# NickDrake117/GNNkeras

Hardware: AMD Instinct MI355X
Metric: node-state updates/s (arcs x iterations / s), forward Loop (higher is better)
Workload: dtype f32; 1 GPU; C4 Erdos-Renyi 1000000 nodes / 10000000 arcs, state_dim=64, max_iteration=50, threshold=0 (k=50), node-focused, average aggregation, BN+Dense(159->64,selu) state net

## Files before the change

gnnkeras_amd/_native.py:

```python
from __future__ import annotations

import ctypes as C
import os
import subprocess

import torch

HERE = os.path.dirname(os.path.abspath(__file__))
CSRC = os.path.join(HERE, 'csrc')
LIB_PATH = os.environ.get('GNNKERAS_AMD_LIB') or os.path.join(CSRC, 'libgnnloop.so')

GNN_ABI_VERSION = 10
GNN_MAX_LAYERS = 8
GNN_MAX_TYPES = 8

ACTIVATIONS = {'linear': 0, None: 0, 'relu': 1, 'selu': 2, 'tanh': 3, 'sigmoid': 4, 'elu': 5, 'softplus': 6,
               'softmax': 7}
FOCUS = {'n': 0, 'a': 1, 'g': 2}
FLAG_UNFUSED = 1
FLAG_NO_EARLY_EXIT = 2
FLAG_FUSED_GEN_MASK = 7 << 4
FLAG_TRAIN_HIDDEN_SMALL = 1 << 8
XC_FILL, XC_VALID = 0, 1
FLAG_FUSED_GEN2, FLAG_FUSED_GEN4, FLAG_FUSED_GEN5, FLAG_FUSED_GEN6, FLAG_FUSED_GEN7 = 2 << 4, 4 << 4, 5 << 4, 6 << 4, 7 << 4

EXPORTS = ['gnn_last_error', 'gnn_last_status', 'gnn_last_kernel_name', 'gnn_abi_version', 'gnn_struct_size', 'gnn_loop_workspace_bytes', 'gnn_loop_forward', 'gnn_loop_groups_supported', 'gnn_loop_group_max_nodes', 'gnn_aggregate',
           'gnn_loop_xc_applies', 'gnn_loop_route_name', 'gnn_train_xc_applies',
           'gnn_mlp_workspace_bytes', 'gnn_mlp_forward', 'gnn_converged', 'gnn_state_step', 'gnn_state_step_agg', 'gnn_state_ld', 'gnn_debug_occupy', 'gnn_debug_occupy_until', 'gnn_debug_expiry_beacon', 'gnn_debug_host_flag',
           'gnn_debug_f4_tile_plan', 'gnn_debug_f4_tile_queue_const', 'gnn_debug_f4_last_tickets',
           'gnn_device_malloc', 'gnn_device_free', 'gnn_ipc_export', 'gnn_ipc_open', 'gnn_ipc_close', 'gnn_shard_iteration_peers', 'gnn_peer_wait', 'gnn_peer_publish', 'gnn_shard_iteration_split_rows',
           'gnn_shard_setup', 'gnn_shard_iteration', 'gnn_shard_output', 'gnn_gather_rows',
           'gnn_shard_can_split', 'gnn_shard_partial', 'gnn_shard_iteration_split',
           'gnn_dense', 'gnn_fold_bn', 'gnn_dense_grad_workspace_bytes', 'gnn_dense_grad', 'gnn_act_grad',
           'gnn_colstats_workspace_bytes', 'gnn_colstats', 'gnn_first_layer_param_grads', 'gnn_bn_input_grad',
           'gnn_scatter_add_rows', 'gnn_axpby', 'gnn_loss_grad', 'gnn_dropout', 'gnn_adam_step', 'gnn_adam_multi', 'gnn_sgd_step',
           'gnn_converged_gated', 'gnn_aggregate_gated', 'gnn_train_workspace_bytes', 'gnn_train_step', 'gnn_train_groups_supported', 'gnn_ragged_copy',
           'gnn_train_step_ex', 'gnn_train_phases_supported', 'gnn_gate_all',
           'gnn_comm_unique_id', 'gnn_comm_create', 'gnn_comm_destroy', 'gnn_shard_loop']
GNN_MAX_SEGMENTS = 6
LOSSES = {'categorical_crossentropy': 0, 'cce': 0, 'binary_crossentropy': 1, 'bce': 1, 'mse': 2,
          'mean_squared_error': 2, 'mae': 3, 'mean_absolute_error': 3}

_f32p = C.POINTER(C.c_float)
_i32p = C.POINTER(C.c_int32)
# ... 200 lines not shown
        l.gnn_shard_iteration_peers.restype = C.c_int
        l.gnn_shard_iteration_peers.argtypes = [C.POINTER(LoopArgs), C.c_void_p, C.c_void_p, C.c_int32, C.c_void_p, C.c_int32, C.c_int32, C.c_void_p, C.c_int32,
                                                C.POINTER(PeerSet)]
        l.gnn_peer_wait.restype = C.c_int
        l.gnn_peer_wait.argtypes = [C.c_void_p, C.c_int32, C.c_int32, C.c_int32, C.c_void_p, C.c_void_p]
        l.gnn_peer_publish.restype = C.c_int
        l.gnn_peer_publish.argtypes = [C.POINTER(PeerSet), C.c_void_p, C.c_void_p, C.c_int64, C.c_int32, C.c_int32, C.c_int32, C.c_void_p]
        l.gnn_debug_host_flag.restype = C.c_int
        l.gnn_debug_host_flag.argtypes = [C.POINTER(C.POINTER(C.c_int32)), C.POINTER(C.c_void_p)]
        l.gnn_debug_f4_tile_plan.restype = None
        l.gnn_debug_f4_tile_plan.argtypes = [C.c_int32, C.c_int32, C.c_int32, C.POINTER(C.c_int32)]
        l.gnn_debug_f4_tile_queue_const.restype = C.c_int32
        l.gnn_debug_f4_tile_queue_const.argtypes = [C.c_int32, C.c_int32]
        l.gnn_debug_f4_last_tickets.restype = C.c_longlong
        l.gnn_debug_f4_last_tickets.argtypes = []
        l.gnn_debug_expiry_beacon.restype = C.c_int
        l.gnn_debug_expiry_beacon.argtypes = [C.POINTER(C.c_void_p), C.c_int32, C.c_void_p]
        l.gnn_state_step_agg.restype = C.c_int
        l.gnn_state_step_agg.argtypes = [C.POINTER(LoopArgs), C.c_void_p, C.c_void_p, C.c_int32, C.c_void_p, C.c_int32, C.c_void_p, C.c_void_p]
        l.gnn_state_ld.restype = C.c_int32
        l.gnn_state_ld.argtypes = [C.c_int32]
        l.gnn_shard_setup.restype = C.c_int
        l.gnn_shard_setup.argtypes = [C.POINTER(LoopArgs)]
        l.gnn_shard_iteration.restype = C.c_int
        l.gnn_shard_iteration.argtypes = [C.POINTER(LoopArgs), C.c_void_p, C.c_void_p, C.c_int32, C.c_void_p, C.c_int32,
                                          C.c_int32, C.c_void_p, C.c_int32]
        l.gnn_shard_output.restype = C.c_int
        l.gnn_shard_output.argtypes = [C.POINTER(LoopArgs), C.c_void_p, C.c_void_p, C.c_int32]
        vp, i32, f32, sz = C.c_void_p, C.c_int32, C.c_float, C.c_size_t
        protos = {
# ... 84 lines not shown
```

gnnkeras_amd/csrc/gnnloop.hip:

```cpp
#include <hip/hip_runtime.h>
#include <stdarg.h>
#include <stddef.h>
#include <stdio.h>
#include <stdlib.h>
#include <string.h>
#include <algorithm>
#include <mutex>
#include <string>
#include <vector>

#include "../../include/gnnloop.h"
#include "kernels_general.hpp"
#include "kernel_state_fused2.hpp"
#include "kernel_state_fused4.hpp"
#include "kernel_state_small.hpp"
#include "kernel_state_mid.hpp"
#include "kernel_state_lds.hpp"
#include "kernel_state_lds_types.hpp"
#include "kernel_state_wide.hpp"
#include "kernels_batch.hpp"
#include "kernels_setup.hpp"
#include "kernel_rowdense.hpp"
#include "kernel_state_xwide.hpp"

// ... 38 lines not shown
    if (S <= 128) {
        int p = 16;
        while (p < S) p <<= 1;
        return p;
    }
    return round_up(S, 4);
}

struct Knobs {
    int pin;
    int flag_pin, env_pin;
    int mid_max_nodes;
    bool prefix_fusion, xwide, rowdense;
    bool xc; int xc_min_nodes;
    bool tile_queue;
};
const Knobs &process_knobs() {
    static const Knobs once = [] {
        Knobs k = {};
        const char *e;
        k.env_pin = (e = getenv("GNN_FUSED_KERNEL")) ? atoi(e) : 0;
        k.mid_max_nodes = (e = getenv("GNN_MID_MAX_NODES")) ? atoi(e) : 36000;
        k.prefix_fusion = !((e = getenv("GNN_PREFIX_FUSION")) && e[0] == '0');
        k.xwide = !((e = getenv("GNN_XWIDE")) && atoi(e) == 0);
        k.rowdense = !((e = getenv("GNN_ROWDENSE")) && e[0] == '0');
        return k;
    }();
    return once;
}
Knobs knobs(int flags) {
    Knobs k = process_knobs();
    k.flag_pin = (flags & GNN_FLAG_FUSED_GEN_MASK) >> 4;
    k.pin = k.flag_pin ? k.flag_pin : k.env_pin;
    const char *e = getenv("GNN_XC"), *m = getenv("GNN_XC_MIN_NODES");
    k.xc = !(e && atoi(e) == 0);
    k.xc_min_nodes = m ? atoi(m) : 196608;
    const char *q = getenv("GNN_F4_TILE_QUEUE");
    k.tile_queue = !(q && atoi(q) == 0);
    return k;
}

struct Carver {
    char *base;
    size_t off = 0;
    explicit Carver(void *b) : base((char *)b) {}
    template <typename T>
    T *take(size_t count) {
        off = (off + 255) & ~(size_t)255;
        T *p = base ? (T *)(base + off) : nullptr;
        off += count * sizeof(T);
        return p;
    }
};
// ... 336 lines not shown
    float *Wx;
    bool xc_ok;
    float *buf[2], *agg;
    float *hid[2]; int ld_hid;
    float *Wf_out, *bf_out;
    float *ohid[2]; int ld_ohid;
    float *out_nodes;
    int *idx_src, *idx_dst;
    size_t bytes;
};

constexpr int GNN_SMALL_MAX_TILES = 512;
constexpr int GNN_LOOP_WORDS = 16 + 32 + gnn::MID_BAR_WORDS;
constexpr int GNN_TQ_WORDS = 8;
inline size_t tq_words(const gnn_loop_args_t &a) { return (size_t)GNN_TQ_WORDS * (size_t)a.max_iteration; }

int state_width(const gnn_loop_args_t &a) { return a.state_dim > 0 ? a.state_dim : a.dim_node_label; }

int make_plan(const gnn_loop_args_t &a, void *ws, Plan &p, bool validate_ptrs) {
    memset(&p, 0, sizeof(p));
    if (a.abi_version != GNN_ABI_VERSION) return fail("abi_version %d != %d", a.abi_version, GNN_ABI_VERSION);
    if (a.n_nodes < 0 || a.n_arcs < 0) return fail("negative graph size");
    if (a.state_dim < 0 || a.max_iteration < 0 || !(a.state_threshold >= 0.0f)) return fail("state_dim, max_iteration, state_threshold must be >= 0");
    p.composite = a.composite != 0;
    p.T = p.composite ? a.n_types : 1;
    if (p.T < 1 || p.T > GNN_MAX_TYPES) return fail("n_types %d out of [1,%d]", p.T, GNN_MAX_TYPES);
    if (p.composite && a.max_iteration < 1) return not_covered("composite GNN requires max_iteration > 0");
    p.N = a.n_nodes; p.E = a.n_arcs; p.L = a.dim_node_label; p.A = a.dim_arc_label;
    p.S = state_width(a);
    if (p.S < 1) return fail("state width is 0 (state_dim == 0 and dim_node_label == 0)");
// ... 75 lines not shown
            TRY(check_csr(a.nodegraph, "nodegraph", a.nodegraph.n_dst, p.M));
        }
        if (a.n_heavy_segments > 0) {
            if (!a.heavy_seg_beg || !a.heavy_seg_end) return fail("heavy_seg_beg / heavy_seg_end is NULL");
            TRY(check_csr(a.adjacency_light, "adjacency_light", p.N, (a.nodes_src ? a.adjacency.n_src : p.N) + a.n_heavy_segments));
        }
        if (p.composite) {
            if (!a.type_nodes && p.N > 0) return fail("type_nodes is NULL");
            if (a.type_offsets[0] != 0 || a.type_offsets[p.T] != p.N) return fail("type_offsets must span [0, n_nodes]");
            for (int t = 0; t < p.T; ++t)
                TRY(check_csr(a.composite_adjacency[t], "composite_adjacency", p.N, a.nodes_src ? a.adjacency.n_src : p.N));
        }
    }

    Carver c(ws);
    p.flags = c.take<int>(a.max_iteration + GNN_LOOP_WORDS + tq_words(a));
    p.err = p.flags ? p.flags + a.max_iteration + 12 : nullptr;
    p.tq = p.flags ? p.flags + a.max_iteration + GNN_LOOP_WORDS : nullptr;
    p.mid_bar = p.flags ? p.flags + ((a.max_iteration + 16 + 31) & ~31) : nullptr;
    p.pred0 = c.take<int>(std::max(GNN_SMALL_MAX_TILES, p.group_tiles));
    p.d_group_tabs = c.take<int>(a.n_groups > 0 ? 4 * ((size_t)a.n_groups + 1) : 0);
    p.set_bar = c.take<unsigned long long>(a.n_groups > 0 ? 2 * (size_t)a.n_groups : 0);
    for (int t = 0; t < p.T; ++t) {
        p.tp[t].Wf = c.take<float>((size_t)a.net_state[t].in_dim * a.net_state[t].units[0]);
        p.tp[t].bf = c.take<float>(a.net_state[t].units[0]);
    }
    p.Wf_out = c.take<float>((size_t)a.net_output.in_dim * a.net_output.units[0]);
    p.bf_out = c.take<float>(a.net_output.units[0]);
    p.agg_arcs = c.take<float>((size_t)p.N * std::max(p.A, 1));
    p.ld_agg_nodes = p.composite ? sum_dt : (a.state_dim > 0 ? p.L : 0);
    p.agg_nodes = c.take<float>((size_t)p.N * std::max(p.ld_agg_nodes, 1));
// ... 114 lines not shown
    LAUNCH_OK();
    return 0;
}
int check_xc_args(const gnn_loop_args_t &a) {
    if (!a.xc) return 0;
    if (((uintptr_t)a.xc & 255) != 0) return fail("xc must be 256-byte aligned");
    if (a.xc_mode != GNN_XC_FILL && a.xc_mode != GNN_XC_VALID) return fail("unknown xc_mode %d", a.xc_mode);
    return 0;
}

int setup_constants(const gnn_loop_args_t &a, const Plan &p, hipStream_t st, bool zero_loop_words = false, bool skip_c = false,
                    const GivenAgg *given = nullptr, bool xc_line = false, bool xc_valid = false) {
    FoldList fl;
    for (int t = 0; t < p.T; ++t) fl.add(a.net_state[t], p.tp[t].Wf, p.tp[t].bf);
    if (a.net_output.kernel[0]) fl.add(a.net_output, p.Wf_out, p.bf_out);
    if (zero_loop_words) { fl.fa.zero_a = p.flags; fl.fa.n_a = a.max_iteration + GNN_LOOP_WORDS + (int)tq_words(a); fl.fa.zero_b = a.k_out; fl.fa.n_b = 1; }
    TRY(launch_fold_list(fl, st));
    if (xc_line) {
        const TypePlan &tp = p.tp[0];
        if (!xc_valid) TRY(fill_constants_line(a, p.N, a.state_dim > 0 ? p.L : 0, p.A, p.Xc, st));
        gnn::PackSegs ps;
        memset(&ps, 0, sizeof(ps));
        ps.n = tp.ncseg;
        for (int s2 = 0; s2 < tp.ncseg && s2 < 3; ++s2) { ps.width[s2] = tp.cseg[s2].width; ps.wrow[s2] = tp.cseg[s2].wrow; }
        const int H = tp.net->units[0];
        gnn::k_pack_wc<<<cdiv(32 * H, 256), 256, 0, st>>>(tp.Wf, tp.bf, H, ps, tp.Wc);
        LAUNCH_OK();
        return 0;
    }
    if (given) {
        if (p.A > 0) TRY(launch_copy2d(nullptr, given->arcs, given->ld_arcs, p.agg_arcs, p.A, p.N, p.A, p.A, st));
// ... 59 lines not shown
    sa.nodes_src = a.nodes_src ? a.nodes_src : a.nodes; sa.ld_nodes_src = a.nodes_src ? a.ld_nodes_src : a.ld_nodes;
    sa.adj = gnn::SetupCsr{a.adjacency.rowptr, a.adjacency.src, a.adjacency.w, a.adjacency.row_scale};
    sa.arc_labels = a.arc_labels; sa.ld_arcs = a.ld_arcs; sa.A = p.A;
    sa.arcnode = gnn::SetupCsr{a.arcnode.rowptr, a.arcnode.src, a.arcnode.w, a.arcnode.row_scale};
    if (a.state_dim > 0) { sa.row_nodes = p.S; sa.row_aggn = 2 * p.S + p.L; sa.row_agga = 2 * p.S + 2 * p.L; }
    else                 { sa.row_agga = 2 * p.S; }
    sa.C = p.C; sa.ldC = p.ldC;
    sa.state0 = a.state_dim > 0 ? a.state0 : a.nodes; sa.ld_s0 = a.state_dim > 0 ? p.S : a.ld_nodes;
    sa.S = p.S; sa.thr = a.state_threshold; sa.pred0 = p.pred0;
    sa.zero_a = p.flags; sa.n_a = a.max_iteration + GNN_LOOP_WORDS; sa.zero_b = a.k_out; sa.n_b = std::max(1, p.n_groups);
    gnn::k_setup_small<<<sa.n_tiles + 1, 256, gnn::setup_small_lds(sa.net.H, 2 * L + p.A, std::max(a.net_state[0].in_dim, a.net_output.in_dim)), st>>>(sa);
    LAUNCH_OK();
    return 0;
}

__device__ long long g_f4_last_tickets;
__global__ void k_fold_error(const int *err, float *k_out, const int *tq, int n_tq) {
    long long s = 0;
    for (int i = threadIdx.x; i < n_tq; i += 64) s += tq[i];
    for (int off = 32; off >= 1; off >>= 1) s += __shfl_xor(s, off, 64);
    if (threadIdx.x == 0) {
        g_f4_last_tickets = s;
        if (*err != 0) *k_out = -1.0e9f;
    }
}

int launch_fold_error(const Plan &p, float *k_out, hipStream_t st, const int *tq = nullptr, int n_tq = 0) {
    if (!k_out || !p.err) return 0;
    k_fold_error<<<1, 64, 0, st>>>(p.err, k_out, tq, n_tq);
    LAUNCH_OK();
    return 0;
}

__global__ void k_arc_endpoints(const int *__restrict__ out_index, const int *__restrict__ arc_src,
                                const int *__restrict__ arc_dst, int M, int *__restrict__ idx_src, int *__restrict__ idx_dst) {
    const int m = blockIdx.x * blockDim.x + threadIdx.x;
    if (m < M) { const int e = out_index[m]; idx_src[m] = arc_src[e]; idx_dst[m] = arc_dst[e]; }
}

int output_stage(const gnn_loop_args_t &a, const Plan &p, hipStream_t st) {
    if (p.M == 0) return 0;
    const bool with_labels = !p.composite && a.state_dim > 0;
    MlpRun r;
    r.mlp = &a.net_output; r.Wf = p.Wf_out; r.bf = p.bf_out;
// ... 71 lines not shown
    r.nseg = 1;
    r.segs[0] = gnn::Seg{p.agg, nullptr, p.SP, (int)m.units[1], 0};
    r.M = p.N;
    r.hid[0] = p.hid[0]; r.hid[1] = p.hid[1]; r.ld_hid = p.ld_hid;
    r.Y = dst; r.ldy = p.SP;
    r.gate = gate;
    if (flag_next) { r.pred_old = src; r.ld_pred = p.SP; r.pred_thr = a.state_threshold; r.pred_flag = flag_next; r.pred_k = k_out; r.pred_kval = k_val; }
    TRY(run_mlp(r, st));
    if (flag_next && !r.pred_fused) TRY(launch_converge(gate, dst, src, p.N, p.S, p.SP, p.SP, a.state_threshold, flag_next, k_out, k_val, st));
    return 0;
}

int iteration_fused(const gnn_loop_args_t &a, const Plan &p, IterKernel kernel, const int *gate, int n_gate, int gate_stride,
                    const float *src, float *dst, int row_base, int *flag_next, float *k_out, float k_val,
                    hipStream_t st, const gnn_csr_t *adj_override = nullptr, const float *agg_init = nullptr,
                    const int *rows_override = nullptr, int count_override = 0, const gnn_peer_set_t *peers = nullptr, int *tile_ctr = nullptr) {
    TRY(launch_heavy(a, p, n_gate == 1 ? gate : nullptr, src, st));
    const gnn_csr_t &adj = adj_override ? *adj_override : iter_adjacency(a, p);
    gnn::Fused2Args fa;
    memset(&fa, 0, sizeof(fa));
    fill_fused_args(fa, a, p, adj);
    fa.gate = n_gate ? gate : nullptr; fa.n_gate = n_gate; fa.gate_stride = gate_stride;
    fa.state_in = src; fa.state_out = dst; fa.row_base = row_base; fa.err = p.err;
    if (rows_override && fa.n_types == 1) {
        fa.tp[0].rows = rows_override; fa.tp[0].count = count_override;
        if (count_override == 0) fa.n_types = 0;
    }
    fa.flag_next = flag_next;
    fa.k_out = k_out; fa.k_val = k_val;
    fa.agg_init = agg_init;
    if (peers) {
        if (peers->n_peers < 0 || peers->n_peers > GNN_MAX_PEERS) return fail("n_peers %d out of [0, %d]", peers->n_peers, GNN_MAX_PEERS);
        fa.n_peers = peers->n_peers;
        for (int i = 0; i < peers->n_peers; ++i) fa.peer_out[i] = peers->state_out_full[i];
    }
    if (p.xc_ok && !adj.w && (agg_init || size_generation(p, a.flags) == 4)) fa.Xc = p.Xc;
    if (tile_ctr && kernel == IterKernel::fused4 && p.T == 1 && fa.n_types == 1 && !rows_override && !agg_init && !peers) fa.tq_ctr = tile_ctr;
    if (fa.n_types == 0) {
        if (k_out) TRY(launch_converge(fa.gate, src, src, 0, p.S, p.SP, p.SP, a.state_threshold, flag_next, k_out, k_val, st));
        return 0;
    }
    if (fa.n_peers > 0 && (p.SP == 128 || p.T != 1 || adj.w || a.net_state[0].n_layers != 1 || (p.SP != 32 && p.SP != 64) || p.n_heavy != 0))
        return fail("peer stores: homogeneous one-layer shards without per-arc weights or hub rows, state widths 17 .. 64");
    if (kernel == IterKernel::wide) FUSED_OK(gnn::launch_wide(fa, device_cus(), st, 0));
    else if (kernel == IterKernel::fused4 || agg_init || fa.n_peers > 0) FUSED_OK(gnn::launch_fused4(fa, p.SP, device_cus(), st));
    else FUSED_OK(gnn::launch_fused2(fa, p.SP, 8, device_cus(), st));
    return 0;
}

int loop_whole(const gnn_loop_args_t &a, const Plan &p, bool mid, const float *first, float *const B[2], const int *pred0,
               int n_pred0, float *state_final, hipStream_t st) {
    gnn::SmallArgs sa;
// ... 251 lines not shown
        B[a.max_iteration & 1] = a.state_out;
    if (a.ev_loop_begin) HIP_OK(hipEventRecord((hipEvent_t)a.ev_loop_begin, st));
    int persistent = 2;
    if (route.whole == WholeLoop::small) {
        persistent = loop_whole(a, p, false, first, B, small_setup ? p.pred0 : nullptr, small_setup ? p.group_tiles : 0, a.state_out, st);
        if (persistent == 1) return 1;
        if (persistent == 2 && small_setup) return fail("whole-loop kernel refused a graph its set-up kernel accepted");
    }
    bool loop_done = persistent == 0;
    if (!loop_done && route.try_mid) {
        const int rc = loop_whole(a, p, true, first, B, nullptr, 0, nullptr, st);
        if (rc == 1) return 1;
        loop_done = rc == 0;
    }
    int *const tq = (!small_setup && knobs(a.flags).tile_queue) ? p.tq : nullptr;
    for (int it = 0; !loop_done && it < a.max_iteration; ++it) {
        const int *gate = no_exit ? nullptr : p.flags + it;
        const float *src = it == 0 ? first : B[it & 1];
        float *dst = B[(it + 1) & 1];
        if (route.iter.fused())                  TRY(iteration_fused(a, p, kernel, gate, gate ? 1 : 0, 0, src, dst, 0, p.flags + it + 1, a.k_out, (float)(it + 1), st,
                                                                     nullptr, nullptr, nullptr, 0, nullptr, tq ? tq + (size_t)GNN_TQ_WORDS * it : nullptr));
        else if (kernel == IterKernel::prefix)   TRY(iteration_prefix(a, p, gate, src, dst, p.flags + it + 1, a.k_out, (float)(it + 1), st));
        else if (kernel == IterKernel::xwide)    TRY(iteration_xwide(a, p, gate, src, dst, p.flags + it + 1, a.k_out, (float)(it + 1), st));
        else                                     TRY(iteration_unfused(a, p, gate, src, dst, 0, p.flags + it + 1, a.k_out, (float)(it + 1), st));
    }

    if (a.ev_loop_end) HIP_OK(hipEventRecord((hipEvent_t)a.ev_loop_end, st));

    if (persistent != 0) {
        const long total = (long)p.N * p.S;
        if (total > 0) {
            gnn::k_select_state<<<std::min(cdiv(total, 256), 256 * 16), 256, 0, st>>>(a.k_out, first, B[0], B[1], p.SP, a.state_out, p.S, p.N, p.S);
            LAUNCH_OK();
        }
    }
    TRY(output_stage(a, p, st));
    if (!loop_done && (route.iter.fused() || kernel == IterKernel::xwide) && a.max_iteration > 0)
        TRY(launch_fold_error(p, a.k_out, st, tq, tq ? (int)tq_words(a) : 0));
    return 0;
}

int gnn_loop_groups_supported(const gnn_loop_args_t *args) {
    if (!args || args->n_groups < 1) return 0;
    Plan p;
    if (make_plan(*args, nullptr, p, false)) return 0;
    const LoopRoute route = route_loop(*args, p);
    if (route.whole == WholeLoop::lds || route.whole == WholeLoop::lds_types) return 2;
    if (p.composite || args->n_groups > GNN_MAX_GROUPS) return 0;
    return route.whole == WholeLoop::small && route.small_setup ? 1 : 0;
}

int gnn_loop_group_max_nodes(const gnn_loop_args_t *args) {
    if (!args) return 0;
// ... 128 lines not shown
        const gnn::F4TilePlan q = gnn::f4_tile_plan(ntiles, n_workgroups, xcd, ahead);
        int32_t *o = out56 + 7 * xcd;
        o[0] = q.t_begin; o[1] = q.t_end; o[2] = q.blk; o[3] = q.T1; o[4] = q.pool_begin; o[5] = q.pool_end; o[6] = q.n_chunks;
    }
}
int32_t gnn_debug_f4_tile_queue_const(int32_t which, int32_t padded_width) {
    switch (which) {
        case 0: return gnn::F4_TQ_CH;
        case 1: return padded_width == 64 ? gnn::Fused4Cfg<64>::AHEAD : padded_width == 32 ? gnn::Fused4Cfg<32>::AHEAD : padded_width == 16 ? gnn::Fused4Cfg<16>::AHEAD : -1;
        case 2: return gnn::F4_TQ_MIN_SHARE;
        case 3: return gnn::F4_TQ_MAX_CHUNKS;
        case 4: return gnn::F4_TQ_TAB;
        default: return -1;
    }
}
long long gnn_debug_f4_last_tickets(void) {
    long long v = -1;
    if (hipDeviceSynchronize() != hipSuccess) return -1;
    return hipMemcpyFromSymbol(&v, HIP_SYMBOL(g_f4_last_tickets), sizeof(v)) == hipSuccess ? v : -1;
}

int gnn_debug_occupy(int32_t n_workgroups, int32_t lds_bytes, int32_t milliseconds, void *stream) {
    if (n_workgroups < 1 || lds_bytes < 0 || lds_bytes > 160 * 1024 || milliseconds < 0 || milliseconds > 10000) return fail("gnn_debug_occupy: bad arguments");
    static bool attr = false;
    if (!attr) { HIP_OK(hipFuncSetAttribute(reinterpret_cast<const void *>(&k_debug_occupy), hipFuncAttributeMaxDynamicSharedMemorySize, 160 * 1024)); attr = true; }
    k_debug_occupy<<<n_workgroups, 64, (size_t)lds_bytes, (hipStream_t)stream>>>((unsigned long long)milliseconds * 100000ull, nullptr, nullptr);
    LAUNCH_OK();
    return 0;
}

// ... 282 lines not shown
```

gnnkeras_amd/csrc/kernel_state_fused2.hpp:

```cpp
#pragma once
#include <hip/hip_runtime.h>
#include "kernels_general.hpp"

namespace gnn {

struct FusedType {
    const int *rows;
    int count;
    const float *Wf;
    int wrow_state, wrow_agg;
    int H, act;
    const float *W2;
    const float *b2;
    int act2;
    const float *Wc;
    int out2;
};

struct Fused2Args {
    const int *gate; int n_gate, gate_stride;
    const int *rowptr, *src;
    const float *w, *row_scale;
    const float *state_in;
    float *state_out;
    int row_base;
    const float *C; int ldC;
    int n_types;
    FusedType tp[GNN_MAX_TYPES];
    int blk_begin[GNN_MAX_TYPES + 1];
    int S;
    float thr;
    int *flag_next;
    float *k_out; float k_val;
    int *err;
    int *tq_ctr;
    const float *Xc;
    const float *agg_init;
    const void *hdr; void *hdr_write;
    float *peer_out[GNN_MAX_PEERS]; int n_peers;
};

inline char *last_kernel_name() { static thread_local char name[96] = ""; return name; }
#define GNN_SET_KERNEL_NAME(...) snprintf(::gnn::last_kernel_name(), 96, __VA_ARGS__)

template <int SP, int TM, int NW>
struct Fused2Cfg {
    static constexpr int NT = 64 * NW;
    static constexpr int LPR = SP / 4;
    static constexpr int NPP = NT / LPR;
    static constexpr int NPASS = TM / NPP;
// ... 323 lines not shown
```

gnnkeras_amd/csrc/kernel_state_fused4.hpp:

```cpp
#pragma once
#include <hip/hip_runtime.h>
#include "kernel_state_fused2.hpp"
#include "buffer_ops.hpp"

namespace gnn {

constexpr int XC_K = 32;

constexpr int F4_TQ_CH = 2;
constexpr int F4_TQ_NUM = 7, F4_TQ_DEN = 8;
constexpr int F4_TQ_TAB = 1024;
constexpr int F4_TQ_MAX_CHUNKS = 960;
constexpr int F4_TQ_MIN_SHARE = 16;
constexpr int F4_TQ_END = -2;
struct F4TilePlan { int t_begin, t_end, blk, T1, pool_begin, pool_end, n_chunks; };
__host__ __device__ inline F4TilePlan f4_tile_plan(int ntiles, int nblk, int xcd, int ahead) {
    F4TilePlan q;
    const int tpx = (ntiles + 7) >> 3;
    q.blk = (nblk + 7 - xcd) >> 3;
    q.t_begin = xcd * tpx < ntiles ? xcd * tpx : ntiles;
    q.t_end = (xcd + 1) * tpx < ntiles ? (xcd + 1) * tpx : ntiles;
    const int n = q.t_end - q.t_begin, b = q.blk > 0 ? q.blk : 1;
    const int n_min = ntiles - 7 * tpx > 0 ? ntiles - 7 * tpx : 0, b_max = (nblk + 7) >> 3;
    const bool queue = (nblk & 7) == 0 && nblk > 0 && n_min >= F4_TQ_MIN_SHARE * b_max && (int)((long)F4_TQ_NUM * n_min / ((long)F4_TQ_DEN * b_max)) >= ahead;
    if (!queue) {
        q.T1 = (n + b - 1) / b; q.pool_begin = q.pool_end = q.t_end; q.n_chunks = 0;
        return q;
    }
    q.T1 = (int)((long)F4_TQ_NUM * n / ((long)F4_TQ_DEN * b));
    if (n - q.T1 * b > F4_TQ_MAX_CHUNKS * F4_TQ_CH) q.T1 = (n - F4_TQ_MAX_CHUNKS * F4_TQ_CH + b - 1) / b;
    q.pool_begin = q.t_begin + q.T1 * b; q.pool_end = q.t_end;
    q.n_chunks = (q.pool_end - q.pool_begin + F4_TQ_CH - 1) / F4_TQ_CH;
    return q;
}

template <int SP, int NC = 4, bool L2 = false, bool XC = false, int VPL = 1, bool TQ = false>
struct Fused4Cfg {
    static constexpr int NW = 16, NT = 64 * NW;
    static constexpr int NCONS = NC;
    static constexpr int NPROD = NW - NCONS;
    static constexpr int LPR = SP / (4 * VPL);
    static constexpr int RPWV = 64 / LPR;
    static constexpr int PPT = 16 / RPWV;
    static constexpr int IPL = 16 / LPR;
    static constexpr int LDX = 2 * SP + 2;
    static constexpr bool SWZ = SP >= 32;
    static constexpr int LDW = SWZ ? SP : SP + 32;
    static constexpr int NCT = SP / 16;
// ... 61 lines not shown
    int *fill = reinterpret_cast<int *>(W2s + Cfg::W2F);
    int *freed = fill + NS;
    int *tab = freed + NS;

    const int tid = threadIdx.x, lane = tid & 63, wave = tid >> 6;
    if (tid == 0) F4_STAMP(0);
    const int S = a.S;
    int ty = 0;
    while (ty + 1 < a.n_types && (int)blockIdx.x >= a.blk_begin[ty + 1]) ++ty;
    const FusedType tp = a.tp[ty];
    const int O2 = tp.out2 > 0 ? tp.out2 : S;
    const int bid = blockIdx.x - a.blk_begin[ty], nblk = a.blk_begin[ty + 1] - a.blk_begin[ty];
    const int count = tp.count;
    const int *__restrict__ rows = tp.rows;

    const int ntiles = (count + 15) / 16;
    const int xcd = bid & 7, lb = bid >> 3;
    const int blk_per_xcd = (nblk + 7 - xcd) >> 3;
    const int tpx = (ntiles + 7) >> 3;
    const int t_end = min(ntiles, (xcd + 1) * tpx);
    const int t_first = xcd * tpx + lb;
    const int T = t_first < t_end ? (t_end - t_first + blk_per_xcd - 1) / blk_per_xcd : 0;
    const F4TilePlan tq = TQ ? f4_tile_plan(ntiles, nblk, xcd, Cfg::AHEAD) : F4TilePlan{};
    int tq_end = F4_TQ_TAB;
    auto tq_entry = [&](int ci) -> int {
        if (ci >= tq_end) return F4_TQ_END;
        int v, spin = 0;
        while ((v = __builtin_amdgcn_readfirstlane(f4_ld_acquire(&tab[ci]))) == 0) {
            if (spin >= SPIN_MAX) { bad = 1; v = F4_TQ_END; break; }
            ++spin; __builtin_amdgcn_s_sleep(1);
        }
        if (v == F4_TQ_END) tq_end = ci;
        return v;
    };
    auto tile_of = [&](int L) -> int {
        if constexpr (!TQ) return L < T ? t_first + L * blk_per_xcd : F4_TQ_END;
        else {
            if (L < tq.T1) return t_first + L * blk_per_xcd;
            const int v = tq_entry((L - tq.T1) / F4_TQ_CH);
            if (v == F4_TQ_END) return F4_TQ_END;
            const int t = v - 1 + (L - tq.T1) % F4_TQ_CH;
            return t < t_end ? t : -1;
        }
    };

    const __amdgpu_buffer_rsrc_t r_C = buf_rsrc(XC ? a.Xc : a.C), r_rows = buf_rsrc(tp.rows), r_state = buf_rsrc(a.state_in),
                                 r_rowptr = buf_rsrc(a.rowptr), r_src = buf_rsrc(a.src), r_w = buf_rsrc(HAS_W ? a.w : nullptr),
                                 r_scale = buf_rsrc(a.row_scale), r_init = buf_rsrc(INIT ? a.agg_init : nullptr);
    const bool has_scale = a.row_scale != nullptr;
    char *__restrict__ obase = reinterpret_cast<char *>(a.state_out);
    int any = 0;

    const int p = wave - Cfg::NCONS;
    const int qr = lane / LPR;
    const int l4 = lane % LPR;
    const int njobs = T * Cfg::PPT;
    auto job_m = [&](int n) -> int {
// ... 85 lines not shown
#ifdef GNN_F4_PROFILE
        const unsigned long long tr_ = f4_now();
#endif
        for (int n = p; TQ ? tlA != F4_TQ_END : n < njobs; n += Cfg::NPROD) {
            const int t = n / Cfg::PPT;
            const int row = (n % Cfg::PPT) * Cfg::RPWV + qr;
            const int j = jA;
            bool draws = false;
            int dci = 0, dprev = 1, ticket = 0;
            if constexpr (TQ) {
                const int x = t + Cfg::AHEAD - tq.T1;
                draws = n % Cfg::PPT == 0 && x >= 0 && x % F4_TQ_CH == 0;
                if (draws) {
                    dci = x / F4_TQ_CH;
                    if (dci > 0) dprev = tq_entry(dci - 1);
                    if (dprev != F4_TQ_END && lane == 0) ticket = atomicAdd(a.tq_ctr + xcd, 1);
                }
            }
#ifdef GNN_F4_PROFILE
            unsigned long long tg_ = f4_now();
#endif
            const int begB = buf_ld_i32(r_rowptr, jB >= 0 ? 4u * (unsigned)jB : BUF_OFF);
            const int endB = buf_ld_i32(r_rowptr, jB >= 0 ? 4u * (unsigned)jB + 4u : BUF_OFF);
            int tlC = 0;
            if constexpr (TQ) tlC = tile_of((n + 2 * Cfg::NPROD) / Cfg::PPT);
            const int jC = node_of(TQ ? job_m_of(tlC, n + 2 * Cfg::NPROD) : job_m(n + 2 * Cfg::NPROD));
            const float scl = buf_ld_f32(r_scale, j >= 0 ? 4u * (unsigned)j : BUF_OFF);
            f32x4 own[VPL], acc[VPL];
#pragma unroll
            for (int x = 0; x < VPL; ++x) {
                own[x] = buf_ld_f32x4(r_state, j >= 0 ? (unsigned)(a.row_base + j) * (unsigned)(SP * 4) + 16u * (unsigned)(VPL * l4 + x) : BUF_OFF);
// ... 46 lines not shown
                    idc[u] = buf_ld_i32(r_src, e < endA ? 4u * (unsigned)e : BUF_OFF);
                    wsc[u] = HAS_W ? buf_ld_f32(r_w, e < endA ? 4u * (unsigned)e : BUF_OFF) : 0.0f;
                }
            }
            if (has_scale) {
#pragma unroll
                for (int x = 0; x < VPL; ++x) acc[x] *= scl;
            }
            jA = jB; begA = begB; endA = endB; jB = jC;
#pragma unroll
            for (int u = 0; u < IPL; ++u) { idsA[u] = idsB[u]; wsA[u] = wsB[u]; }
            if constexpr (TQ) {
                tlA = tlB; tlB = tlC;
                if (draws) {
                    const int tk = __builtin_amdgcn_readfirstlane(ticket);
                    const int v = (dprev == F4_TQ_END || tk >= tq.n_chunks) ? F4_TQ_END : tq.pool_begin + tk * F4_TQ_CH + 1;
                    if (lane == 0 && dci < F4_TQ_TAB) __hip_atomic_store(&tab[dci], v, __ATOMIC_RELEASE, __HIP_MEMORY_SCOPE_WORKGROUP);
                }
            }

            const int s = t % NS, round = t / NS;
#ifdef GNN_F4_PROFILE
            if (lane == 0) atomicAdd(&g_f4_prof[0], f4_now() - tg_);
            tg_ = f4_now();
#endif
            {
                int spin = 0;
                while (__builtin_amdgcn_readfirstlane(f4_ld_acquire(&freed[s])) < round) {
                    if (spin >= SPIN_MAX) { bad = 1; break; }
                    ++spin; __builtin_amdgcn_s_sleep(1);
                }
// ... 246 lines not shown
    if (PEERS)
        GNN_SET_KERNEL_NAME("k_state_fused4<%d,%s,%d,%d,%s,%s,%s,%d,%s,true> (peer stores)", SP, HAS_W ? "true" : "false", DEPTH, NC, L2 ? "true" : "false", INIT ? "true" : "false", XC ? "true" : "false", VPL, HDR ? "true" : "false");
    else if (VPL == 1 && !HDR)
        GNN_SET_KERNEL_NAME("k_state_fused4<%d,%s,%d,%d,%s,%s,%s>", SP, HAS_W ? "true" : "false", DEPTH, NC, L2 ? "true" : "false", INIT ? "true" : "false", XC ? "true" : "false");
    else
        GNN_SET_KERNEL_NAME("k_state_fused4<%d,%s,%d,%d,%s,%s,%s,%d,%s>", SP, HAS_W ? "true" : "false", DEPTH, NC, L2 ? "true" : "false", INIT ? "true" : "false", XC ? "true" : "false", VPL, HDR ? "true" : "false");
    k_state_fused4<SP, HAS_W, DEPTH, NC, L2, INIT, XC, VPL, HDR, PEERS, TQ><<<grid, Cfg::NT, Cfg::LDS_BYTES, st>>>(fa);
    return hipGetLastError() == hipSuccess ? 0 : 1;
}

template <int SP, bool HAS_W, bool L2, bool XC>
int launch_fused4_plain(Fused2Args &fa, int n_cu, hipStream_t st) {
    if constexpr (SP == 64 && !HAS_W && !L2) {
        if (fa.tq_ctr && fa.n_types == 1 && !fa.tp[0].rows) {
            const int ntiles = (fa.tp[0].count + 15) / 16;
            if (f4_tile_plan(ntiles, fused4_blocks(ntiles, ntiles, 2 * n_cu), 7, Fused4Cfg<SP, 4, L2, XC, 1, true>::AHEAD).n_chunks > 0)
                return launch_fused4_one<SP, HAS_W, 4, L2, 4, false, XC, 1, false, false, true>(fa, n_cu, st);
        }
    }
    fa.tq_ctr = nullptr;
    return launch_fused4_one<SP, HAS_W, 4, L2, 4, false, XC>(fa, n_cu, st);
}

inline int launch_fused4(Fused2Args &fa, int SP, int n_cu, hipStream_t st) {
    if (fa.n_peers > 0) {
        if (fa.w || fa.tp[0].W2 || (SP != 32 && SP != 64)) return 1;
#define F4_PEER(SPV)                                                                                                               \
        if (SP == SPV) {                                                                                                           \
            if (fa.agg_init) return fa.Xc ? launch_fused4_one<SPV, false, 4, false, 4, true, true, 1, false, true>(fa, n_cu, st)   \
                                          : launch_fused4_one<SPV, false, 4, false, 4, true, false, 1, false, true>(fa, n_cu, st); \
            return fa.Xc ? launch_fused4_one<SPV, false, 4, false, 4, false, true, 1, false, true>(fa, n_cu, st)                   \
                         : launch_fused4_one<SPV, false, 4, false, 4, false, false, 1, false, true>(fa, n_cu, st);                 \
        }
        F4_PEER(32)
        F4_PEER(64)
// ... 25 lines not shown
```

include/gnnloop.h:

```cpp
#ifndef GNNLOOP_H
#define GNNLOOP_H

#include <stddef.h>
#include <stdint.h>

#ifdef __cplusplus
extern "C" {
#endif

#define GNN_ABI_VERSION 10

enum gnn_activation {
    GNN_ACT_LINEAR = 0, GNN_ACT_RELU = 1, GNN_ACT_SELU = 2, GNN_ACT_TANH = 3, GNN_ACT_SIGMOID = 4,
    GNN_ACT_ELU = 5, GNN_ACT_SOFTPLUS = 6, GNN_ACT_SOFTMAX = 7
};

enum gnn_focus { GNN_FOCUS_NODE = 0, GNN_FOCUS_ARC = 1, GNN_FOCUS_GRAPH = 2 };

enum gnn_flags {
    GNN_FLAG_UNFUSED = 1,
    GNN_FLAG_NO_EARLY_EXIT = 2,
    GNN_FLAG_FUSED_GEN2 = 2 << 4, GNN_FLAG_FUSED_GEN4 = 4 << 4,
    GNN_FLAG_FUSED_GEN5 = 5 << 4, GNN_FLAG_FUSED_GEN6 = 6 << 4, GNN_FLAG_FUSED_GEN7 = 7 << 4, GNN_FLAG_FUSED_GEN_MASK = 7 << 4,
    GNN_FLAG_TRAIN_HIDDEN_SMALL = 1 << 8
// ... 102 lines not shown
int gnn_converged(const float *state, const float *state_old, int32_t n, int32_t dim, int32_t ld, float threshold,
                  int32_t *flag, void *stream);

int gnn_state_step(const gnn_loop_args_t *args, const float *state_in, float *state_out, int32_t *flag_out);

int gnn_state_step_agg(const gnn_loop_args_t *args, const float *state_in, const float *aggregated_nodes, int32_t ld_aggregated_nodes,
                       const float *aggregated_arcs, int32_t ld_aggregated_arcs, float *state_out, int32_t *flag_out);

int gnn_debug_occupy(int32_t n_workgroups, int32_t lds_bytes, int32_t milliseconds, void *stream);
int gnn_debug_occupy_until(int32_t n_workgroups, int32_t lds_bytes, int32_t max_milliseconds, const int32_t *release_flag, void *stream);
int gnn_debug_host_flag(int32_t **host_out, int32_t **dev_out);
int gnn_debug_expiry_beacon(int32_t **beacon_out, int32_t reset, void *stream);
void gnn_debug_f4_tile_plan(int32_t ntiles, int32_t n_workgroups, int32_t ahead, int32_t *out56);
int32_t gnn_debug_f4_tile_queue_const(int32_t which, int32_t padded_width);
long long gnn_debug_f4_last_tickets(void);

int32_t gnn_state_ld(int32_t state_width);
int gnn_gather_rows(const float *src, int32_t ld_src, const int32_t *idx, int32_t M, int32_t width, float *dst,
                    int32_t ld_dst, void *stream);
int gnn_shard_setup(const gnn_loop_args_t *args);
int gnn_shard_iteration(const gnn_loop_args_t *args, const float *state_in_full, float *state_out_full,
                        int32_t row_base, const int32_t *gate, int32_t n_gate, int32_t gate_stride, int32_t *flag_out,
                        int32_t iteration);
int gnn_shard_output(const gnn_loop_args_t *args, const float *buf0_full, const float *buf1_full, int32_t row_base);
int gnn_shard_can_split(const gnn_loop_args_t *args);
int gnn_shard_partial(const gnn_loop_args_t *args, const gnn_csr_t *adjacency_own, const float *state_in_full,
                      float *agg_partial);
int gnn_shard_iteration_split(const gnn_loop_args_t *args, const gnn_csr_t *adjacency_halo, const float *agg_partial,
                              const float *state_in_full, float *state_out_full, int32_t row_base, const int32_t *gate,
                              int32_t n_gate, int32_t gate_stride, int32_t *flag_out, int32_t iteration);
// ... 201 lines not shown
```

Measured before the change: 22.10 billion arc-updates/s.

## Add cross-XCD shared tile pool for fused4 dynamic tile queue

```diff
diff --git a/gnnkeras_amd/_native.py b/gnnkeras_amd/_native.py
--- a/gnnkeras_amd/_native.py
+++ b/gnnkeras_amd/_native.py
@@ -27,7 +27,7 @@
 EXPORTS = ['gnn_last_error', 'gnn_last_status', 'gnn_last_kernel_name', 'gnn_abi_version', 'gnn_struct_size', 'gnn_loop_workspace_bytes', 'gnn_loop_forward', 'gnn_loop_groups_supported', 'gnn_loop_group_max_nodes', 'gnn_aggregate',
            'gnn_loop_xc_applies', 'gnn_loop_route_name', 'gnn_train_xc_applies',
            'gnn_mlp_workspace_bytes', 'gnn_mlp_forward', 'gnn_converged', 'gnn_state_step', 'gnn_state_step_agg', 'gnn_state_ld', 'gnn_debug_occupy', 'gnn_debug_occupy_until', 'gnn_debug_expiry_beacon', 'gnn_debug_host_flag',
-           'gnn_debug_f4_tile_plan', 'gnn_debug_f4_tile_queue_const', 'gnn_debug_f4_last_tickets',
+           'gnn_debug_f4_tile_plan', 'gnn_debug_f4_tile_queue_const', 'gnn_debug_f4_last_tickets', 'gnn_debug_f4_shared_plan', 'gnn_debug_f4_last_shared_tickets',
            'gnn_device_malloc', 'gnn_device_free', 'gnn_ipc_export', 'gnn_ipc_open', 'gnn_ipc_close', 'gnn_shard_iteration_peers', 'gnn_peer_wait', 'gnn_peer_publish', 'gnn_shard_iteration_split_rows',
            'gnn_shard_setup', 'gnn_shard_iteration', 'gnn_shard_output', 'gnn_gather_rows',
            'gnn_shard_can_split', 'gnn_shard_partial', 'gnn_shard_iteration_split',
@@ -258,6 +258,10 @@
         l.gnn_debug_f4_tile_queue_const.argtypes = [C.c_int32, C.c_int32]
         l.gnn_debug_f4_last_tickets.restype = C.c_longlong
         l.gnn_debug_f4_last_tickets.argtypes = []
+        l.gnn_debug_f4_shared_plan.restype = None
+        l.gnn_debug_f4_shared_plan.argtypes = [C.c_int32, C.c_int32, C.c_int32, C.POINTER(C.c_int32)]
+        l.gnn_debug_f4_last_shared_tickets.restype = C.c_longlong
+        l.gnn_debug_f4_last_shared_tickets.argtypes = []
         l.gnn_debug_expiry_beacon.restype = C.c_int
         l.gnn_debug_expiry_beacon.argtypes = [C.POINTER(C.c_void_p), C.c_int32, C.c_void_p]
         l.gnn_state_step_agg.restype = C.c_int
diff --git a/gnnkeras_amd/csrc/gnnloop.hip b/gnnkeras_amd/csrc/gnnloop.hip
--- a/gnnkeras_amd/csrc/gnnloop.hip
+++ b/gnnkeras_amd/csrc/gnnloop.hip
@@ -76,6 +76,7 @@
     bool prefix_fusion, xwide, rowdense;
     bool xc; int xc_min_nodes;
     bool tile_queue;
+    bool shared_pool;
 };
 const Knobs &process_knobs() {
     static const Knobs once = [] {
@@ -99,6 +100,8 @@
     k.xc_min_nodes = m ? atoi(m) : 196608;
     const char *q = getenv("GNN_F4_TILE_QUEUE");
     k.tile_queue = !(q && atoi(q) == 0);
+    const char *g = getenv("GNN_F4_SHARED_POOL");
+    k.shared_pool = k.tile_queue && !(g && atoi(g) == 0);
     return k;
 }
 
@@ -465,6 +468,7 @@
 constexpr int GNN_LOOP_WORDS = 16 + 32 + gnn::MID_BAR_WORDS;
 constexpr int GNN_TQ_WORDS = 8;
 inline size_t tq_words(const gnn_loop_args_t &a) { return (size_t)GNN_TQ_WORDS * (size_t)a.max_iteration; }
+inline size_t tq_shared_words(const gnn_loop_args_t &a) { return (size_t)a.max_iteration; }
 
 int state_width(const gnn_loop_args_t &a) { return a.state_dim > 0 ? a.state_dim : a.dim_node_label; }
 
@@ -570,7 +574,7 @@
     }
 
     Carver c(ws);
-    p.flags = c.take<int>(a.max_iteration + GNN_LOOP_WORDS + tq_words(a));
+    p.flags = c.take<int>(a.max_iteration + GNN_LOOP_WORDS + tq_words(a) + tq_shared_words(a));
     p.err = p.flags ? p.flags + a.max_iteration + 12 : nullptr;
     p.tq = p.flags ? p.flags + a.max_iteration + GNN_LOOP_WORDS : nullptr;
     p.mid_bar = p.flags ? p.flags + ((a.max_iteration + 16 + 31) & ~31) : nullptr;
@@ -715,7 +719,7 @@
     FoldList fl;
     for (int t = 0; t < p.T; ++t) fl.add(a.net_state[t], p.tp[t].Wf, p.tp[t].bf);
     if (a.net_output.kernel[0]) fl.add(a.net_output, p.Wf_out, p.bf_out);
-    if (zero_loop_words) { fl.fa.zero_a = p.flags; fl.fa.n_a = a.max_iteration + GNN_LOOP_WORDS + (int)tq_words(a); fl.fa.zero_b = a.k_out; fl.fa.n_b = 1; }
+    if (zero_loop_words) { fl.fa.zero_a = p.flags; fl.fa.n_a = a.max_iteration + GNN_LOOP_WORDS + (int)tq_words(a) + (int)tq_shared_words(a); fl.fa.zero_b = a.k_out; fl.fa.n_b = 1; }
     TRY(launch_fold_list(fl, st));
     if (xc_line) {
         const TypePlan &tp = p.tp[0];
@@ -805,20 +809,22 @@
     return 0;
 }
 
-__device__ long long g_f4_last_tickets;
-__global__ void k_fold_error(const int *err, float *k_out, const int *tq, int n_tq) {
-    long long s = 0;
+__device__ long long g_f4_last_tickets, g_f4_last_shared_tickets;
+__global__ void k_fold_error(const int *err, float *k_out, const int *tq, int n_tq, int n_shared) {
+    long long s = 0, g = 0;
     for (int i = threadIdx.x; i < n_tq; i += 64) s += tq[i];
-    for (int off = 32; off >= 1; off >>= 1) s += __shfl_xor(s, off, 64);
+    for (int i = threadIdx.x; i < n_shared; i += 64) g += tq[n_tq + i];
+    for (int off = 32; off >= 1; off >>= 1) { s += __shfl_xor(s, off, 64); g += __shfl_xor(g, off, 64); }
     if (threadIdx.x == 0) {
         g_f4_last_tickets = s;
+        g_f4_last_shared_tickets = g;
         if (*err != 0) *k_out = -1.0e9f;
     }
 }
 
-int launch_fold_error(const Plan &p, float *k_out, hipStream_t st, const int *tq = nullptr, int n_tq = 0) {
+int launch_fold_error(const Plan &p, float *k_out, hipStream_t st, const int *tq = nullptr, int n_tq = 0, int n_shared = 0) {
     if (!k_out || !p.err) return 0;
-    k_fold_error<<<1, 64, 0, st>>>(p.err, k_out, tq, n_tq);
+    k_fold_error<<<1, 64, 0, st>>>(p.err, k_out, tq, n_tq, n_shared);
     LAUNCH_OK();
     return 0;
 }
@@ -920,7 +926,8 @@
 int iteration_fused(const gnn_loop_args_t &a, const Plan &p, IterKernel kernel, const int *gate, int n_gate, int gate_stride,
                     const float *src, float *dst, int row_base, int *flag_next, float *k_out, float k_val,
                     hipStream_t st, const gnn_csr_t *adj_override = nullptr, const float *agg_init = nullptr,
-                    const int *rows_override = nullptr, int count_override = 0, const gnn_peer_set_t *peers = nullptr, int *tile_ctr = nullptr) {
+                    const int *rows_override = nullptr, int count_override = 0, const gnn_peer_set_t *peers = nullptr, int *tile_ctr = nullptr,
+                    int *shared_ctr = nullptr) {
     TRY(launch_heavy(a, p, n_gate == 1 ? gate : nullptr, src, st));
     const gnn_csr_t &adj = adj_override ? *adj_override : iter_adjacency(a, p);
     gnn::Fused2Args fa;
@@ -941,7 +948,7 @@
         for (int i = 0; i < peers->n_peers; ++i) fa.peer_out[i] = peers->state_out_full[i];
     }
     if (p.xc_ok && !adj.w && (agg_init || size_generation(p, a.flags) == 4)) fa.Xc = p.Xc;
-    if (tile_ctr && kernel == IterKernel::fused4 && p.T == 1 && fa.n_types == 1 && !rows_override && !agg_init && !peers) fa.tq_ctr = tile_ctr;
+    if (tile_ctr && kernel == IterKernel::fused4 && p.T == 1 && fa.n_types == 1 && !rows_override && !agg_init && !peers) { fa.tq_ctr = tile_ctr; fa.tq_shared = shared_ctr; }
     if (fa.n_types == 0) {
         if (k_out) TRY(launch_converge(fa.gate, src, src, 0, p.S, p.SP, p.SP, a.state_threshold, flag_next, k_out, k_val, st));
         return 0;
@@ -1223,12 +1230,13 @@
         loop_done = rc == 0;
     }
     int *const tq = (!small_setup && knobs(a.flags).tile_queue) ? p.tq : nullptr;
+    int *const tq_shared = (tq && knobs(a.flags).shared_pool) ? tq + tq_words(a) : nullptr;
     for (int it = 0; !loop_done && it < a.max_iteration; ++it) {
         const int *gate = no_exit ? nullptr : p.flags + it;
         const float *src = it == 0 ? first : B[it & 1];
         float *dst = B[(it + 1) & 1];
         if (route.iter.fused())                  TRY(iteration_fused(a, p, kernel, gate, gate ? 1 : 0, 0, src, dst, 0, p.flags + it + 1, a.k_out, (float)(it + 1), st,
-                                                                     nullptr, nullptr, nullptr, 0, nullptr, tq ? tq + (size_t)GNN_TQ_WORDS * it : nullptr));
+                                                                     nullptr, nullptr, nullptr, 0, nullptr, tq ? tq + (size_t)GNN_TQ_WORDS * it : nullptr, tq_shared ? tq_shared + it : nullptr));
         else if (kernel == IterKernel::prefix)   TRY(iteration_prefix(a, p, gate, src, dst, p.flags + it + 1, a.k_out, (float)(it + 1), st));
         else if (kernel == IterKernel::xwide)    TRY(iteration_xwide(a, p, gate, src, dst, p.flags + it + 1, a.k_out, (float)(it + 1), st));
         else                                     TRY(iteration_unfused(a, p, gate, src, dst, 0, p.flags + it + 1, a.k_out, (float)(it + 1), st));
@@ -1245,7 +1253,7 @@
     }
     TRY(output_stage(a, p, st));
     if (!loop_done && (route.iter.fused() || kernel == IterKernel::xwide) && a.max_iteration > 0)
-        TRY(launch_fold_error(p, a.k_out, st, tq, tq ? (int)tq_words(a) : 0));
+        TRY(launch_fold_error(p, a.k_out, st, tq, tq ? (int)tq_words(a) : 0, tq ? (int)tq_shared_words(a) : 0));
     return 0;
 }
 
@@ -1404,6 +1412,15 @@
         default: return -1;
     }
 }
+void gnn_debug_f4_shared_plan(int32_t ntiles, int32_t n_workgroups, int32_t ahead, int32_t *out3) {
+    const gnn::F4SharedPlan s = gnn::f4_shared_plan(ntiles, n_workgroups, ahead);
+    out3[0] = s.G; out3[1] = s.first; out3[2] = s.n_chunks;
+}
+long long gnn_debug_f4_last_shared_tickets(void) {
+    long long v = -1;
+    if (hipDeviceSynchronize() != hipSuccess) return -1;
+    return hipMemcpyFromSymbol(&v, HIP_SYMBOL(g_f4_last_shared_tickets), sizeof(v)) == hipSuccess ? v : -1;
+}
 long long gnn_debug_f4_last_tickets(void) {
     long long v = -1;
     if (hipDeviceSynchronize() != hipSuccess) return -1;
diff --git a/gnnkeras_amd/csrc/kernel_state_fused2.hpp b/gnnkeras_amd/csrc/kernel_state_fused2.hpp
--- a/gnnkeras_amd/csrc/kernel_state_fused2.hpp
+++ b/gnnkeras_amd/csrc/kernel_state_fused2.hpp
@@ -34,6 +34,8 @@
     float *k_out; float k_val;
     int *err;
     int *tq_ctr;
+    int *tq_shared;
+    int tq_shared_tiles;
     const float *Xc;
     const float *agg_init;
     const void *hdr; void *hdr_write;
diff --git a/gnnkeras_amd/csrc/kernel_state_fused4.hpp b/gnnkeras_amd/csrc/kernel_state_fused4.hpp
--- a/gnnkeras_amd/csrc/kernel_state_fused4.hpp
+++ b/gnnkeras_amd/csrc/kernel_state_fused4.hpp
@@ -32,6 +32,28 @@
     q.pool_begin = q.t_begin + q.T1 * b; q.pool_end = q.t_end;
     q.n_chunks = (q.pool_end - q.pool_begin + F4_TQ_CH - 1) / F4_TQ_CH;
     return q;
+}
+
+constexpr int F4_SP_DEN = 64;
+constexpr int F4_TQ_SHARED = 1 << 30;
+struct F4SharedPlan { int G, first, n_chunks; };
+__host__ __device__ inline F4SharedPlan f4_shared_plan(int ntiles, int nblk, int ahead) {
+    F4SharedPlan s = {0, ntiles, 0};
+    if (f4_tile_plan(ntiles, nblk, 7, ahead).n_chunks == 0) return s;
+    const int b_max = (nblk + 7) >> 3, tpx = (ntiles + 7) >> 3;
+    const int xcd_chunks = (tpx / 8 + b_max) / F4_TQ_CH + 1;
+    const int room = (F4_TQ_MAX_CHUNKS - 1 - xcd_chunks) * F4_TQ_CH - 7;
+    int want = ntiles / F4_SP_DEN;
+    if (want > room) want = room;
+    if (want < 1) return s;
+    int m = (ntiles - want) & ~7;
+    if (f4_tile_plan(m, nblk, 7, ahead).n_chunks == 0) {
+        m = (ntiles - 1) & ~7;
+        if (f4_tile_plan(m, nblk, 7, ahead).n_chunks == 0) return s;
+    }
+    s.G = ntiles - m; s.first = m;
+    s.n_chunks = (s.G + F4_TQ_CH - 1) / F4_TQ_CH;
+    return s;
 }
 
 template <int SP, int NC = 4, bool L2 = false, bool XC = false, int VPL = 1, bool TQ = false>
@@ -123,7 +145,10 @@
     const int count = tp.count;
     const int *__restrict__ rows = tp.rows;
 
-    const int ntiles = (count + 15) / 16;
+    const int ntiles_all = (count + 15) / 16;
+    const int sp_G = TQ ? a.tq_shared_tiles : 0;
+    const F4SharedPlan sp = {sp_G, ntiles_all - sp_G, (sp_G + F4_TQ_CH - 1) / F4_TQ_CH};
+    const int ntiles = ntiles_all - sp.G;
     const int xcd = bid & 7, lb = bid >> 3;
     const int blk_per_xcd = (nblk + 7 - xcd) >> 3;
     const int tpx = (ntiles + 7) >> 3;
@@ -148,8 +173,8 @@
             if (L < tq.T1) return t_first + L * blk_per_xcd;
             const int v = tq_entry((L - tq.T1) / F4_TQ_CH);
             if (v == F4_TQ_END) return F4_TQ_END;
-            const int t = v - 1 + (L - tq.T1) % F4_TQ_CH;
-            return t < t_end ? t : -1;
+            const int t = (v & (F4_TQ_SHARED - 1)) - 1 + (L - tq.T1) % F4_TQ_CH;
+            return t < ((v & F4_TQ_SHARED) ? ntiles_all : t_end) ? t : -1;
         }
     };
 
@@ -265,7 +290,8 @@
                 if (draws) {
                     dci = x / F4_TQ_CH;
                     if (dci > 0) dprev = tq_entry(dci - 1);
-                    if (dprev != F4_TQ_END && lane == 0) ticket = atomicAdd(a.tq_ctr + xcd, 1);
+                    int *const ctr = (dprev & F4_TQ_SHARED) ? a.tq_shared : a.tq_ctr + xcd;
+                    if (dprev != F4_TQ_END && lane == 0) ticket = atomicAdd(ctr, 1);
                 }
             }
 #ifdef GNN_F4_PROFILE
@@ -342,7 +368,14 @@
                 tlA = tlB; tlB = tlC;
                 if (draws) {
                     const int tk = __builtin_amdgcn_readfirstlane(ticket);
-                    const int v = (dprev == F4_TQ_END || tk >= tq.n_chunks) ? F4_TQ_END : tq.pool_begin + tk * F4_TQ_CH + 1;
+                    int v;
+                    if (dprev == F4_TQ_END) v = F4_TQ_END;
+                    else if (dprev & F4_TQ_SHARED) v = tk < sp.n_chunks ? F4_TQ_SHARED | (sp.first + tk * F4_TQ_CH + 1) : F4_TQ_END;
+                    else if (tk >= tq.n_chunks && sp.G > 0) {
+                        const int tk2 = __builtin_amdgcn_readfirstlane(lane == 0 ? atomicAdd(a.tq_shared, 1) : 0);
+                        v = tk2 < sp.n_chunks ? F4_TQ_SHARED | (sp.first + tk2 * F4_TQ_CH + 1) : F4_TQ_END;
+                    }
+                    else v = tk < tq.n_chunks ? tq.pool_begin + tk * F4_TQ_CH + 1 : F4_TQ_END;
                     if (lane == 0 && dci < F4_TQ_TAB) __hip_atomic_store(&tab[dci], v, __ATOMIC_RELEASE, __HIP_MEMORY_SCOPE_WORKGROUP);
                 }
             }
@@ -619,11 +652,16 @@
     if constexpr (SP == 64 && !HAS_W && !L2) {
         if (fa.tq_ctr && fa.n_types == 1 && !fa.tp[0].rows) {
             const int ntiles = (fa.tp[0].count + 15) / 16;
-            if (f4_tile_plan(ntiles, fused4_blocks(ntiles, ntiles, 2 * n_cu), 7, Fused4Cfg<SP, 4, L2, XC, 1, true>::AHEAD).n_chunks > 0)
+            constexpr int AHEAD = Fused4Cfg<SP, 4, L2, XC, 1, true>::AHEAD;
+            const int nblk = fused4_blocks(ntiles, ntiles, 2 * n_cu);
+            if (f4_tile_plan(ntiles, nblk, 7, AHEAD).n_chunks > 0) {
+                fa.tq_shared_tiles = fa.tq_shared ? f4_shared_plan(ntiles, nblk, AHEAD).G : 0;
+                if (fa.tq_shared_tiles == 0) fa.tq_shared = nullptr;
                 return launch_fused4_one<SP, HAS_W, 4, L2, 4, false, XC, 1, false, false, true>(fa, n_cu, st);
-        }
-    }
-    fa.tq_ctr = nullptr;
+            }
+        }
+    }
+    fa.tq_ctr = fa.tq_shared = nullptr; fa.tq_shared_tiles = 0;
     return launch_fused4_one<SP, HAS_W, 4, L2, 4, false, XC>(fa, n_cu, st);
 }
 
diff --git a/include/gnnloop.h b/include/gnnloop.h
--- a/include/gnnloop.h
+++ b/include/gnnloop.h
@@ -140,6 +140,8 @@
 void gnn_debug_f4_tile_plan(int32_t ntiles, int32_t n_workgroups, int32_t ahead, int32_t *out56);
 int32_t gnn_debug_f4_tile_queue_const(int32_t which, int32_t padded_width);
 long long gnn_debug_f4_last_tickets(void);
+void gnn_debug_f4_shared_plan(int32_t ntiles, int32_t n_workgroups, int32_t ahead, int32_t *out3);
+long long gnn_debug_f4_last_shared_tickets(void);
 
 int32_t gnn_state_ld(int32_t state_width);
 int gnn_gather_rows(const float *src, int32_t ld_src, const int32_t *idx, int32_t M, int32_t width, float *dst,
```

Measured after the change: 22.30 billion arc-updates/s, median of 6. About the same (+0.9%).
